# laboshinl/loam_velodyne

Hardware: AMD Instinct MI355X
Metric: sweeps/sec (64-ring, 1M-pt map): feature extraction + odometry + scan-to-map registration (higher is better)
Workload: dtype f32

## Files before the change

### loam_velodyne_amd/csrc/odometry.hip

```cpp
#include "odometry.hpp"
#include "odom_schedule.hpp"
#include "pinned_copy.hpp"
#include <chrono>
#include <cstring>
#include <type_traits>

namespace loamx {

constexpr int OD_THREADS = 256;
constexpr int OD_TR_STRIDE = OD_THREADS + 2;
constexpr int OD_PART_STRIDE = 2 * (2 * 16 * LX_NSUM) + 16;
[[maybe_unused]] constexpr int OD_PART_TS = 2 * (2 * 16 * LX_NSUM);

__device__ inline void sincos_f(float a, float& s, float& c) { sincosf(a, &s, &c); }

__device__ inline void transform_to_start(const float* T, float scan_period, const float4 pi, float& x, float& y, float& z) {
  const float s = (1.f / scan_period) * (pi.w - (float)(int)pi.w);
  x = pi.x - s * T[3];
  y = pi.y - s * T[4];
  z = pi.z - s * T[5];
  float sx, cx, sy, cy, sz, cz;
  sincos_f(-s * T[0], sx, cx);
  sincos_f(-s * T[1], sy, cy);
  sincos_f(-s * T[2], sz, cz);
  rot_z(x, y, cz, sz);
  rot_x(y, z, cx, sx);
  rot_y(x, z, cy, sy);
}

// ... 668 lines not shown
              hm->stats = stt;
              hm->done = done_now;
            }
          }
        }
      }
      LM_TS(9);
    }
    __syncthreads();
    if (sh_done) break;
  }
}

#pragma clang diagnostic pop

__device__ inline float4 to_end_point(float4 p, const ToEndParams& P) {
  const float s = (1.f / P.scan_period) * (p.w - (float)(int)p.w);
  float x = p.x - s * P.T[3], y = p.y - s * P.T[4], z = p.z - s * P.T[5];
  float sx, cx, sy, cy, sz, cz;
  sincos_f(-s * P.T[0], sx, cx);
  sincos_f(-s * P.T[1], sy, cy);
  sincos_f(-s * P.T[2], sz, cz);
  rot_z(x, y, cz, sz); rot_x(y, z, cx, sx); rot_y(x, z, cy, sy);
  rot_y(x, z, P.cT[1], P.sT[1]); rot_x(y, z, P.cT[0], P.sT[0]); rot_z(x, y, P.cT[2], P.sT[2]);
  x += P.T[3] - P.shift[0];
  y += P.T[4] - P.shift[1];
  z += P.T[5] - P.shift[2];
  rot_z(x, y, P.c_start[2], P.s_start[2]); rot_x(y, z, P.c_start[0], P.s_start[0]); rot_y(x, z, P.c_start[1], P.s_start[1]);
  rot_y(x, z, P.c_end[1], -P.s_end[1]); rot_x(y, z, P.c_end[0], -P.s_end[0]); rot_z(x, y, P.c_end[2], -P.s_end[2]);
  return make_float4(x, y, z, (float)(int)p.w);
}
__global__ __launch_bounds__(256) void k_transform_to_end_copy(float4* __restrict__ dst, const float4* __restrict__ src, uint32_t n, ToEndParams P) {
  const uint32_t i = blockIdx.x * blockDim.x + threadIdx.x;
  if (i >= n) return;
  dst[i] = to_end_point(src[i], P);
}
__global__ __launch_bounds__(256) void k_transform_to_end(float4* __restrict__ pts, uint32_t n, ToEndParams P) {
  const uint32_t i = blockIdx.x * blockDim.x + threadIdx.x;
  if (i >= n) return;
  pts[i] = to_end_point(pts[i], P);
}
__global__ void k_te_patch(const OdomProblem* __restrict__ probs, uint32_t na, ToEndParams* __restrict__ te) {
  const uint32_t a = blockIdx.x * blockDim.x + threadIdx.x;
  if (a >= na) return;
  const OdomProblem& pb = probs[a];
  ToEndParams& P = te[pb.stream_id];
// ... 701 lines not shown
```

### loam_velodyne_amd/csrc/odometry.hpp

```cpp
#pragma once
#include "common.h"
#include "host_math.h"
#include "registration.hpp"
#include <atomic>
#include <condition_variable>
#include <functional>
#include <mutex>
#include <thread>

namespace loamx {

struct OdomParams {
  float scan_period = 0.1f;
  int max_iterations = 25;
  float delta_t_abort = 0.1f, delta_r_abort = 0.1f;
};

struct OdomStats {
  int iterations, sel, frame, degenerate;
};

struct ToEndParams;

struct OdomProblem {
  const float4* sharp; uint32_t n_sharp;
  const float4* flat; uint32_t n_flat;
  const float4* last_corner; uint32_t n_last_corner;
  const float4* last_surf; uint32_t n_last_surf;
  const float4* sorted;
  const uint32_t* cell_table;
  const GridDescB* lc_desc;
  const GridDescB* ls_desc;
  int* ind;
  float transform[6];
  OdomStats stats;
  int done;
  float matP[36];
// ... 2 lines not shown
  OdomProblem* host_mirror;
  unsigned ticket;
  unsigned xchg_epoch;
  double* part;
  const uint32_t* rf_corner;
  const uint32_t* rf_surf;
  uint32_t rf_epoch;
  uint32_t* err_word;
};

struct OdomInput {
  const float4* sharp; uint32_t n_sharp;
  const float4* less_sharp; uint32_t n_less_sharp;
  const float4* flat; uint32_t n_flat;
  const float4* less_flat; uint32_t n_less_flat;
};

struct ToEndParams {
  float T[6];
  float sT[3], cT[3];
  float shift[3];
  float s_start[3], c_start[3];
  float s_end[3], c_end[3];
  float scan_period;
  int enabled;
};

constexpr int OD_RF_N = 320;

struct ReprojectProbe {
  int variant;
  float4* pts; uint32_t n;
  const uint32_t* d_off; const uint32_t* h_off; uint32_t K, ns;
  const ToEndParams* d_params; const ToEndParams* h_params;
  const float4* src; const float4* src_s; uint32_t n_corner_all;
  uint32_t* bounds; uint32_t* ring_first; uint32_t rf_epoch;
  const float4* const* table; const uint32_t* sid;
};
void reproject_probe_launch(const ReprojectProbe& a, hipStream_t st);

// ... 112 lines not shown
```

### loam_velodyne_amd/csrc/pipeline.hip

```cpp
#include "pinned_copy.hpp"
#include "features.hpp"
#include "odometry.hpp"
#include "registration.hpp"
#include "hostlink.hpp"
#include "densemap.hpp"
#include "odom_lookahead.hpp"
#include <atomic>
#include <deque>
#include <chrono>
#include <mutex>
#include <memory>

namespace loamx {

struct OdomPub {
  HTwist transform, transform_sum;
  OdomStats stats = {0, 0, 0, 0};
  int rc = LOAMX_SKIPPED;
  const float4* last_corner = nullptr; uint32_t n_last_corner = 0;
  const float4* last_surf = nullptr; uint32_t n_last_surf = 0;
  ToEndParams to_end;
};

struct PipeStreamState {
// ... 75 lines not shown
  uint32_t n_groups = 1;
  std::vector<std::unique_ptr<OdomChain>> chains;
  OdomChain& chain_of(uint32_t s) { uint32_t g = 0; while (g + 1 < n_groups && s >= chains[g]->s1) g++; return *chains[g]; }
  OdometryBatch& OB(uint32_t s) { return *chain_of(s).ob; }
  uint32_t LS(uint32_t s) { return s - chain_of(s).s0; }
  loamx_scanreg_config fcfg;
  uint32_t n_streams_;
  int device;
  std::vector<PipeStreamState> st;
  std::vector<std::unique_ptr<FeatureExtractor>> fx;
  static constexpr uint32_t RING = 8;
  bool streaming = false;
  std::atomic<uint32_t> staged_hi{0};
  hipStream_t cstream = nullptr, dstream = nullptr;
  hipEvent_t ev_stage[RING] = {};
  hipEvent_t ev_reg_done = nullptr, ev_d2h[2] = {nullptr, nullptr};
  bool d2h_pending[2] = {false, false};
  uint64_t downloads_direct = 0, downloads_hip = 0;
  HostLinkDma hostlink;
  HostLinkUp uplink;
  uint32_t up_runs[RING] = {};
  std::atomic<long> last_step{-1};
  std::vector<uint32_t> last_full_off;
  std::vector<uint32_t> last_who;
  struct RawSlot {
    bool raw = false, finalized = true;
    std::vector<uint32_t> count, off;
    DevBuf<char> d_bytes;
    DevBuf<float4> d_raw4, d_binned;
    DevBuf<uint32_t> d_ring_fld;
// ... 58 lines not shown
  float feat_ms[OR] = {};
  int f_hi = -1;
  int ahead_depth = std::max(1, std::min(diag_env("LOAMX_ODOM_AHEAD") ? atoi(diag_env("LOAMX_ODOM_AHEAD")) : 6, OR - 2));
  int depth() const { return !prefetch ? 0 : (streaming ? std::min(ahead_depth, (int)RING - 2) : ahead_depth); }
  float last_ms[4] = {0, 0, 0, 0};
  std::atomic<bool> timing{false};

  std::vector<OdomPub> ores[OR];
  std::unique_ptr<LookAhead> la;
  void run_chain_step(OdomChain& c, uint32_t k) {
    const auto tc0 = std::chrono::steady_clock::now();
    c.tr[0] = tr_us(); run_odometry(c, k); c.tr[3] = tr_us();
    c.last_us.store((float)std::chrono::duration<double, std::micro>(std::chrono::steady_clock::now() - tc0).count(), std::memory_order_relaxed);
  }
  int drain_lookahead() { return prefetch ? la->drain() : la->done_min(); }
  void park_odometry(int restart) {
    if (restart >= 0) pre_t = -1;
    la->park(restart);
  }

  ~Pipeline() {
    la.reset();
    for (auto& c : chains) {
      for (auto& e : c->ev_tail) if (e) (void)hipEventDestroy(e);
      for (auto& tm : c->tm) tm.destroy();
    }
    fx.clear();
    for (auto& a : evF) for (auto& e : a) if (e) (void)hipEventDestroy(e);
    for (auto& tm : tmM) tm.destroy();
    for (auto& e : ev_stage) if (e) (void)hipEventDestroy(e);
    for (auto& r : rawslot) if (r.ev_ingest) (void)hipEventDestroy(r.ev_ingest);
    for (auto& e : ev_d2h) if (e) (void)hipEventDestroy(e);
    if (ev_reg_done) (void)hipEventDestroy(ev_reg_done);
    if (cstream) { (void)hipStreamSynchronize(cstream); (void)hipStreamDestroy(cstream); }
    if (dstream) { (void)hipStreamSynchronize(dstream); (void)hipStreamDestroy(dstream); }
    if (fstream) (void)hipStreamDestroy(fstream);
  }

  void launch_features(uint32_t t) {
    TraceRange trace_range("loamx:features");
    finalize_raw(t);
    FeatureExtractor& F = FX(t);
    const uint32_t ns = n_streams_, nring = F.total_rings();
    if (streaming) {
      LX_HIP(hipStreamWaitEvent(fstream, ev_stage[t % RING], 0));
// ... 6 lines not shown
    F.run_async();
    LX_REQUIRE(F.n_offsets() == 3 * (ns + 1) + nring + 1, "internal: offset table layout");
    store_to_pinned_u32(hb.p, F.d_offsets(), F.n_offsets(), fstream);
    LX_HIP(hipEventRecord(evF[t % OR][1], fstream));
    LA(t) = 1;
  }

  std::unique_ptr<FeatureExtractor> new_extractor_() {
    auto f = std::make_unique<FeatureExtractor>(device, fstream);
    f->params = feat_params_from(fcfg);
    return f;
  }
  void feature_stream_() {
    if (!fstream) fstream = create_stream(env_priority("LOAMX_PRIO_FEAT", -1), diag_env("LOAMX_FEAT_CU_STRIDE") ? atoi(diag_env("LOAMX_FEAT_CU_STRIDE")) : 0, 1);
    LX_HIP(hipStreamSynchronize(fstream));
    fx.clear();
  }
  void restart_input_(uint32_t n_slots, bool ring) {
    streaming = ring;
    staged_hi = 0;
    last_step = -1;
    launched.assign(n_slots, 0);
    la->reset();
    f_hi = -1;
  }

  void upload(uint32_t n_steps, const loamx_cloud* clouds, const uint32_t* const* ring_size, const uint32_t* n_rings) {
    LX_REQUIRE(n_steps >= 1 && clouds && ring_size && n_rings, "invalid argument");
    LX_HIP(hipSetDevice(device));
    feature_stream_();
// ... 1 lines not shown
    for (uint32_t t = 0; t < n_steps; t++) {
      auto f = new_extractor_();
      f->upload(n_streams_, clouds + (size_t)t * n_streams_, ring_size + (size_t)t * n_streams_, n_rings + (size_t)t * n_streams_);
      fx.push_back(std::move(f));
    }
  }

  void begin_staging_(uint32_t t, const char* entry) {
    LX_HIP(hipSetDevice(device));
    if (!streaming) {
      LX_REQUIRE(t == 0, "streaming input starts at step 0");
      feature_stream_();
      for (uint32_t k = 0; k < RING; k++) fx.push_back(new_extractor_());
      if (!cstream) cstream = create_stream(0);
      for (auto& e : ev_stage) if (!e) LX_HIP(hipEventCreateWithFlags(&e, hipEventDisableTiming));
      restart_input_(RING, true);
    }
    LX_REQUIRE(t == staged_hi.load(), "steps must be staged in order");
    LX_REQUIRE(t < RING || last_step.load() + (long)RING >= (long)t, std::string(entry) + "(t) needs step(t - 8) to have run: only eight steps can be in flight");
  }
  void publish_staged_(uint32_t t) {
    LA(t) = 0;
    staged_hi.store(t + 1, std::memory_order_release);
  }

  void stage_step(uint32_t t, const loamx_cloud* clouds, const uint32_t* const* ring_size, const uint32_t* n_rings) {
    LX_REQUIRE(clouds && ring_size && n_rings, "invalid argument");
    begin_staging_(t, "stage_step");
    TraceRange trace_range("loamx:pipeline:stage_step");
    if (t > 0) finalize_raw(t - 1);
    rawslot[t % RING].raw = false;
    rawslot[t % RING].finalized = true;
    static const bool direct = !(diag_env("LOAMX_H2D_DIRECT") && atoi(diag_env("LOAMX_H2D_DIRECT")) == 0);
    const int slot = (int)(t % RING);
// ... 233 lines not shown
    for (auto& tm : c.tm)
      if (tm.resolve()) c.ms.store(tm.ms, std::memory_order_relaxed);
    for (uint32_t s = c.s0; s < c.s1; s++) {
      const uint32_t l = s - c.s0;
      OdomStream& O = odom.stream_state(l);
      OdomPub& N = ores[slot][s];
      N.transform = O.transform;
      N.transform_sum = O.transform_sum;
      N.stats = O.stats;
      N.rc = rc[l];
      N.last_corner = odom.d_last_corner(l); N.n_last_corner = O.n_last_corner;
      N.last_surf = odom.d_last_surf(l); N.n_last_surf = O.n_last_surf;
      N.to_end = odom.to_end_params(l, true);
    }
  }
  int pre_t = -1;
  void prestage_gather(int tn, int last_staged, hipStream_t s_) {
    static const bool off = !(diag_env("LOAMX_PRESTAGE") && atoi(diag_env("LOAMX_PRESTAGE")) != 0);
    if (off || !prefetch || pre_t == tn || tn > last_staged || tn < 1) return;
    const uint32_t ns = n_streams_;
    if (la->done_min() < tn) return;
    FeatureExtractor& F = FX((uint32_t)tn);
    std::vector<const float4*> fsrc;
    std::vector<uint32_t> nfr;
    std::vector<ToEndParams> tep;
    for (uint32_t s = 0; s < ns; s++) {
      const OdomPub& N = ores[tn % OR][s];
      if (N.rc != LOAMX_OK) continue;
      fsrc.push_back(F.d_cloud() + F.point_base(s));
      nfr.push_back(F.point_base(s + 1) - F.point_base(s));
      tep.push_back(N.to_end);
    }
    const uint32_t nw = (uint32_t)fsrc.size();
    if (!nw) return;
    const int par = (int)(run_count & 1);
    hostlink.wait(par);
    if (d2h_pending[par]) { LX_HIP(hipStreamWaitEvent(s_, ev_d2h[par], 0)); d2h_pending[par] = false; }
    float4* dst = reg.stage_full_next(nw, nfr.data());
    if (!dst) return;
    std::vector<uint32_t> foff(nw + 1, 0);
    for (uint32_t k = 0; k < nw; k++) foff[k + 1] = foff[k] + nfr[k];
    chains[0]->ob->to_end_gather(dst, foff.data(), fsrc.data(), tep.data(), nw, s_);
    pre_t = tn;
  }

  bool trace = getenv("LOAMX_PIPE_TRACE") != nullptr;
  std::chrono::steady_clock::time_point tr0, tr_exit = std::chrono::steady_clock::now();
  double tr_us() const { return std::chrono::duration<double, std::micro>(std::chrono::steady_clock::now() - tr0).count(); }

  struct Step {
    uint32_t t = 0;
    int ti = 0, last_staged = -1;
    LookaheadWindow w;
    bool late_pending = false;
    hipStream_t s_ = nullptr;
    std::vector<uint32_t> who;
    std::vector<const float4*> cl, sl, fsrc;
    std::vector<uint32_t> ncl, nsl, nfr;
    std::vector<float> guess;
    std::vector<ToEndParams> to_end;
// ... 57 lines not shown
      const uint32_t k = (uint32_t)S.who.size();
      S.cl[k] = P.cur.last_corner; S.ncl[k] = P.cur.n_last_corner;
      S.sl[k] = P.cur.last_surf; S.nsl[k] = P.cur.n_last_surf;
      S.fsrc[k] = F.d_cloud() + F.point_base(s);
      S.nfr[k] = F.point_base(s + 1) - F.point_base(s);
      S.to_end.push_back(P.cur.to_end);
      S.who.push_back(s);
    }
    S.nw = (uint32_t)S.who.size();
  }
  void stage_full_res_(Step& S) {
    if (!S.nw) { last_full_off.clear(); last_who.clear(); return; }
    const uint32_t nw = S.nw;
    std::vector<uint32_t> foff(nw + 1, 0);
    for (uint32_t k = 0; k < nw; k++) foff[k + 1] = foff[k] + S.nfr[k];
    const bool adopted = pre_t == S.ti && reg.adopt_full_next(nw, S.nfr.data());
    pre_t = -1;
    if (!adopted) {
      if (reg.double_buffer_full) {
        const int par = (int)(run_count & 1);
        const double tw0 = trace ? tr_us() : 0.0;
        hostlink.wait(par);
        if (trace) S.tr[4] = tr_us() - tw0;
        if (d2h_pending[par]) { LX_HIP(hipStreamWaitEvent(S.s_, ev_d2h[par], 0)); d2h_pending[par] = false; }
      }
      float4* full_dst = reg.stage_full(nw, S.nfr.data());
      chains[0]->ob->to_end_gather(full_dst, foff.data(), S.fsrc.data(), S.to_end.data(), nw, S.s_);
    }
    last_full_off = foff;
    last_who = S.who;
    run_count++;
  }
  void enqueue_registration_(Step& S) {
    if (!S.nw) return;
    const uint32_t nw = S.nw;
    const RawSlot& R = rawslot[S.t % RING];
    reg.upload_device(nw, S.cl.data(), S.ncl.data(), S.sl.data(), S.nsl.data(), nullptr, nullptr, S.guess.data());
    bool blend = false;
    static const bool no_blend = diag_env("LOAMX_NO_MAP_IMU_BLEND") != nullptr;
    if (!no_blend && streaming && R.raw && !R.scan_time.empty())
      for (uint32_t k = 0; k < nw; k++) blend = blend || R.map_imu_upto[S.who[k]] > 0;
    reg.defer_full = blend;
    reg.on_first_wait = [&]() { release_late_(S); prestage_gather(S.ti + 1, S.last_staged, S.s_); };
    reg.run_async();
    reg.on_first_wait = nullptr;
    if (blend) {
      std::vector<float> p6(6 * (size_t)nw);
      reg.download(p6.data(), nullptr);
      if (reg.submap_sufficient())
        for (uint32_t k = 0; k < nw; k++)
          (void)map_imu_blend(S.who[k], R.map_imu_upto[S.who[k]], R.scan_time[S.who[k]], fcfg.scan_period, &p6[6 * (size_t)k]);
      reg.finish_with_poses(p6.data());
      reg.defer_full = false;
    }
    if (reg.double_buffer_full) {
      if (!ev_reg_done) LX_HIP(hipEventCreateWithFlags(&ev_reg_done, hipEventDisableTiming));
      LX_HIP(hipEventRecord(ev_reg_done, S.s_));
    }
  }
  void release_behind_registration_(Step& S) {
    release_late_(S);
    if (S.nw) prestage_gather(S.ti + 1, S.last_staged, S.s_);
    if (timing) tmM[S.t & 1].stop(S.s_);
    S.tr[1] = tr_us();
  }
  int collect_(Step& S) {
    int ret = LOAMX_SKIPPED;
    if (S.nw) {
      std::vector<float> poses(6 * (size_t)S.nw);
      std::vector<SweepStats> ss(S.nw);
      reg.download(poses.data(), nullptr);
      reg.download_stats(ss.data());
      for (uint32_t k = 0; k < S.nw; k++) {
        PipeStreamState& P = st[S.who[k]];
        P.map_stats = ss[k];
        P.mapped = true;
        if (reg.submap_sufficient()) {
// ... 292 lines not shown
```

### loam_velodyne_amd/csrc/registration.hip

```cpp
#include "registration.hpp"
#include "pinned_copy.hpp"
#include <atomic>
#include <chrono>
#include "scan.hpp"
#include "voxel.hpp"

namespace loamx {

__global__ __launch_bounds__(256) void k_stack(const float4* __restrict__ in, const float4* const* __restrict__ src, uint32_t n,
                                               const uint32_t* __restrict__ seg_off, uint32_t nseg, const Pose* __restrict__ poses,
                                               float inv_corner, float inv_surf, float4* __restrict__ stack, int* __restrict__ ijk,
                                               int* __restrict__ seg_minmax) {
  const uint32_t i = blockIdx.x * blockDim.x + threadIdx.x;
  const bool active = i < n;
  uint32_t seg = 0;
  int ix = 0, iy = 0, iz = 0;
  if (active) {
    seg = vox_find_seg(seg_off, nseg, i);
    const Pose T = poses[seg >> 1];
    const float4 p = src ? src[seg][i - seg_off[seg]] : in[i];
    float x = p.x, y = p.y, z = p.z;
    to_map(T, x, y, z);
    to_be_mapped(T, x, y, z);
    stack[i] = make_float4(x, y, z, p.w);
// ... 462 lines not shown
  const float4 p = queries[q];
  unsigned long long wk[6];
  uint32_t win[6];
  knn5_group<KNN_LPQ, QB>(*desc, pts, cell_start, p.x, p.y, p.z, gl, tab + grp, wk, win);
  if (gl != 0) return;
#pragma unroll
  for (int j = 0; j < 5; j++) {
    idx5[5 * (size_t)q + j] = wk[j] != KNN_NONE ? (uint32_t)(wk[j] & 0xffffffffull) : 0xffffffffu;
    d2_5[5 * (size_t)q + j] = wk[j] != KNN_NONE ? __uint_as_float((uint32_t)(wk[j] >> 32)) : FLT_MAX;
  }
}

__global__ __launch_bounds__(256) void k_transform_full(float4* __restrict__ full, uint32_t n, const uint32_t* __restrict__ full_off,
                                                        uint32_t ns, const Pose* __restrict__ poses, const SweepStats* __restrict__ stats,
                                                        uint32_t* __restrict__ full_done, int mode, uint32_t tag,
                                                        const uint32_t* __restrict__ skip_word, uint32_t skip_value) {
  uint32_t i = blockIdx.x * blockDim.x + threadIdx.x;
  if (i >= n) return;
  if (skip_word && *skip_word == skip_value) return;
  const uint32_t s = vox_find_seg(full_off, ns, i);
  if (mode == 1) {
    if (!stats[s].done) return;
    if (i == full_off[s]) full_done[s] = tag;
  } else if (mode == 2) {
    if (full_done[s] != 0u) return;
  }
  const Pose T = poses[s];
  float4 p = full[i];
  to_map(T, p.x, p.y, p.z);
  full[i] = p;
}

__global__ __launch_bounds__(256) void k_gather_segments(float4* __restrict__ dst, const uint32_t* __restrict__ off, uint32_t nseg,
                                                         const float4* const* __restrict__ src, uint32_t n) {
  const uint32_t i = blockIdx.x * blockDim.x + threadIdx.x;
  if (i >= n) return;
  const uint32_t k = vox_find_seg(off, nseg, i);
  dst[i] = src[k][i - off[k]];
}

struct ParamBlock1 { uint32_t w[18]; };
__global__ __launch_bounds__(256) void k_gather_one(float4* __restrict__ dst, const float4* __restrict__ src, uint32_t n, ParamBlock1 blk,
                                                    uint32_t* __restrict__ blk_dst) {
// ... 109 lines not shown
  LX_HIP(hipStreamWaitEvent(st_, ev_build_, 0));
  LX_HIP(hipEventRecord(ev_swap_, st_));
  corner_index.swap(corner_next_);
  surf_index.swap(surf_next_);
  corner_index.bind(st_);
  surf_index.bind(st_);
  next_staged_ = false;
  swapped_once_ = true;
}

template <class Count> static void prefix_offsets(std::vector<uint32_t>& off, uint32_t n, Count&& count) {
  off.assign(n + 1, 0);
  for (uint32_t s = 0; s < n; s++) off[s + 1] = off[s] + count(s);
}

template <class Count> void Registrar::plan_inputs_(uint32_t n_sweeps, bool staged, Count&& count) {
  LX_REQUIRE(n_sweeps >= 1 && n_sweeps <= max_sweeps_, "n_sweeps out of range for this handle");
  LX_HIP(hipSetDevice(device_));
  n_sweeps_ = n_sweeps;
  h_seg_off_.assign(2 * n_sweeps + 1, 0);
  if (!staged) h_full_off_.assign(n_sweeps + 1, 0);
  max_q_per_sweep_ = 0;
  for (uint32_t s = 0; s < n_sweeps; s++) {
    const uint32_t nc = count(s, 0), nf = count(s, 1);
    h_seg_off_[2 * s + 1] = h_seg_off_[2 * s] + nc;
    h_seg_off_[2 * s + 2] = h_seg_off_[2 * s + 1] + nf;
    max_q_per_sweep_ = std::max(max_q_per_sweep_, nc + nf);
    if (!staged) h_full_off_[s + 1] = h_full_off_[s] + count(s, 2);
  }
  n_in_ = h_seg_off_[2 * n_sweeps];
  if (!staged) n_full_ = h_full_off_[n_sweeps];
  in_.reserve(n_in_ + 1);
  stack_.reserve(n_in_ + 1);
  ds_pts_.reserve(n_in_ + 1);
  vox_.reserve(n_in_ + 1, 2 * n_sweeps);
  LX_REQUIRE(n_in_ < SCAN_MAX_N, "too many feature points in one batch");
  if (n_full_) full_.reserve(n_full_);
  nblk_ = max_q_per_sweep_ / GN_TILE + 2;
  partials_.reserve((size_t)n_sweeps * nblk_ * LX_NSUM);
}

size_t Registrar::write_param_block_(const float* guess6, const float4* const* corner_src, const float4* const* surf_src, const float4* const* full_src) {
  const uint32_t ns = n_sweeps_;
  const size_t nseg = 2 * (size_t)ns;
  const size_t o_off = sizeof(float) * 6 * ns, o_full = o_off + sizeof(uint32_t) * (nseg + 1);
  const size_t end_full = o_full + sizeof(uint32_t) * (ns + 1), o_src = (end_full + 15) & ~(size_t)15;
  const size_t bytes = corner_src ? o_src + sizeof(float4*) * (nseg + ns) : end_full;
  h_blob_.reserve(bytes + 16);
  blob_.reserve(bytes + 16);
  memcpy(h_blob_.p, guess6, sizeof(float) * 6 * ns);
  memcpy(h_blob_.p + o_off, h_seg_off_.data(), sizeof(uint32_t) * (nseg + 1));
  memcpy(h_blob_.p + o_full, h_full_off_.data(), sizeof(uint32_t) * (ns + 1));
  if (corner_src) {
    const float4** hsrc = (const float4**)(h_blob_.p + o_src);
    for (uint32_t s = 0; s < ns; s++) { hsrc[2 * s] = corner_src[s]; hsrc[2 * s + 1] = surf_src[s]; }
    for (uint32_t s = 0; s < ns; s++) hsrc[nseg + s] = full_src ? full_src[s] : nullptr;
  }
  d_guess_ = (const float*)blob_.p;
  d_seg_off_ = (const uint32_t*)(blob_.p + o_off);
  d_full_off_ = (const uint32_t*)(blob_.p + o_full);
  d_src_ = corner_src ? (const float4* const*)(blob_.p + o_src) : nullptr;
  return bytes;
}

void Registrar::upload(uint32_t n_sweeps, const loamx_cloud* corner_last, const loamx_cloud* surf_last, const loamx_cloud* full_res,
                       const float* guess6, bool wait) {
  LX_REQUIRE(corner_last && surf_last && guess6, "NULL input");
  plan_inputs_(n_sweeps, false, [&](uint32_t s, int k) {
    const loamx_cloud* c = k == 0 ? &corner_last[s] : k == 1 ? &surf_last[s] : full_res ? &full_res[s] : nullptr;
    if (!c) return 0u;
    check_cloud(c, false);
    return c->count;
  });
  h_in_.reserve(n_in_ + 1);
  for (uint32_t s = 0; s < n_sweeps; s++) {
    pack_cloud(&corner_last[s], h_in_.p + h_seg_off_[2 * s]);
    pack_cloud(&surf_last[s], h_in_.p + h_seg_off_[2 * s + 1]);
  }
  if (!packed_all_finite(h_in_.p, n_in_)) throw Error(LOAMX_E_INVALID, "a feature cloud holds non-finite coordinates");
  fetch_from_pinned(in_.p, h_in_.p, n_in_, st_);
  if (n_full_) {
    h_full_.reserve(n_full_);
    for (uint32_t s = 0; s < n_sweeps; s++) pack_cloud(&full_res[s], h_full_.p + h_full_off_[s]);
    fetch_from_pinned(full_.p, h_full_.p, n_full_, st_);
  }
  const size_t bytes = write_param_block_(guess6, nullptr, nullptr, nullptr);
  LX_HIP(hipMemcpyAsync(blob_.p, h_blob_.p, bytes, hipMemcpyHostToDevice, st_));
  if (wait) LX_HIP(hipStreamSynchronize(st_));
}

float4* Registrar::stage_full(uint32_t n_sweeps, const uint32_t* n_full) {
  LX_REQUIRE(n_sweeps >= 1 && n_sweeps <= max_sweeps_, "n_sweeps out of range for this handle");
  full_next_staged_ = false;
  prefix_offsets(h_full_off_, n_sweeps, [&](uint32_t s) { return n_full[s]; });
  n_full_ = h_full_off_[n_sweeps];
  if (double_buffer_full) {
    std::swap(full_.p, full_alt_.p);
    std::swap(full_.cap, full_alt_.cap);
  }
  full_.reserve((size_t)n_full_ + 1);
  full_staged_ = true;
  return full_.p;
}

float4* Registrar::stage_full_next(uint32_t n_sweeps, const uint32_t* n_full) {
  LX_REQUIRE(double_buffer_full, "internal: pre-staging needs the second full-resolution buffer");
  LX_REQUIRE(n_sweeps >= 1 && n_sweeps <= max_sweeps_, "n_sweeps out of range for this handle");
  prefix_offsets(next_full_off_, n_sweeps, [&](uint32_t s) { return n_full[s]; });
  if ((size_t)next_full_off_[n_sweeps] + 1 > full_alt_.cap) return nullptr;
  full_next_staged_ = true;
  return full_alt_.p;
}
bool Registrar::adopt_full_next(uint32_t n_sweeps, const uint32_t* n_full) {
  if (!full_next_staged_ || next_full_off_.size() != n_sweeps + 1) { full_next_staged_ = false; return false; }
  for (uint32_t s = 0; s < n_sweeps; s++)
    if (next_full_off_[s + 1] - next_full_off_[s] != n_full[s]) { full_next_staged_ = false; return false; }
  full_next_staged_ = false;
  h_full_off_ = next_full_off_;
  n_full_ = h_full_off_[n_sweeps];
  std::swap(full_.p, full_alt_.p);
  std::swap(full_.cap, full_alt_.cap);
  full_staged_ = true;
  return true;
}

void Registrar::upload_device(uint32_t n_sweeps, const float4* const* corner_last, const uint32_t* n_corner,
                              const float4* const* surf_last, const uint32_t* n_surf, const float4* const* full_res,
                              const uint32_t* n_full, const float* guess6) {
  const bool staged = full_staged_ && !full_res;
  full_staged_ = false;
  plan_inputs_(n_sweeps, staged, [&](uint32_t s, int k) { return k == 0 ? n_corner[s] : k == 1 ? n_surf[s] : full_res ? n_full[s] : 0u; });
  const size_t bytes = write_param_block_(guess6, corner_last, surf_last, full_res);
  if (n_sweeps == 1 && n_full_ && !staged && bytes == sizeof(ParamBlock1)) {
    ParamBlock1 pb1;
    memcpy(pb1.w, h_blob_.p, sizeof(pb1));
    hipLaunchKernelGGL(k_gather_one, dim3((n_full_ + 255) / 256), dim3(256), 0, st_, full_.p, full_res[0], n_full_, pb1, (uint32_t*)blob_.p);
  } else {
    LX_HIP(hipMemcpyAsync(blob_.p, h_blob_.p, bytes, hipMemcpyHostToDevice, st_));
    if (n_full_ && !staged)
      hipLaunchKernelGGL(k_gather_segments, dim3((n_full_ + 255) / 256), dim3(256), 0, st_, full_.p, d_full_off_, n_sweeps, d_src_ + 2 * (size_t)n_sweeps,
                         n_full_);
  }
}

static double host_us() {
  return std::chrono::duration<double, std::micro>(std::chrono::steady_clock::now().time_since_epoch()).count();
}
struct Registrar::RunTrace {
  bool on;
  double t0, front = 0, first_gn = 0, callback = 0;
  int looks = 0;
};
#ifdef LOAMX_PROF_GN
static DevBuf<unsigned long long> g_gn_dbg;
#endif

void Registrar::enqueue_full(int mode) {
  if (!n_full_) return;
  if (mode == 1 && ++full_tag_ == 0u) full_tag_ = 1u;
  const uint32_t* skip = run_.vb_unchecked ? vb_.d_fail_word() : nullptr;
  hipLaunchKernelGGL(k_transform_full, dim3((n_full_ + 255) / 256), dim3(256), 0, st_, full_.p, n_full_, d_full_off_, n_sweeps_, poses_.p,
                     stats_.p, full_done_.p, mode, full_tag_, skip, vb_.epoch());
}

void Registrar::enqueue_front(bool legacy) {
  const uint32_t ns = n_sweeps_, nseg = 2 * ns, n = n_in_;
  if (legacy || n == 0)
    hipLaunchKernelGGL(k_pose_init, dim3((ns + 63) / 64), dim3(64), 0, st_, d_guess_, ns, poses_.p, stats_.p, vox_.seg_minmax(), arrive_.p,
                       full_done_.p);
  if (n == 0) {
    LX_HIP(hipMemsetAsync(ds_off_.p, 0, sizeof(uint32_t) * (nseg + 1), st_));
    return;
  }
  if (legacy) {
    const uint32_t nb = (n + 255) / 256;
    hipLaunchKernelGGL(k_stack, dim3(nb), dim3(256), 0, st_, in_.p, d_src_, n, d_seg_off_, nseg, poses_.p, 1.0f / params.corner_leaf,
                       1.0f / params.surf_leaf, stack_.p, vox_.ijk(), vox_.seg_minmax());
// ... 416 lines not shown
```

### loam_velodyne_amd/csrc/registration.hpp

```cpp
#pragma once
#include <functional>
#include "common.h"
#include "dev_math.hpp"
#include "reg_schedule.hpp"
#include "submap_index.hpp"
#include "voxel.hpp"
#include "voxbucket.hpp"

namespace loamx {

constexpr int LX_RES_THREADS = 256;
constexpr int LX_NSUM = 28;

struct SweepStats {
  int iterations, sel, corner_q, surf_q, degenerate, done, pad0, pad1;
};

__host__ __device__ inline int mirror_check_word(const SweepStats& st, const Pose& T) {
  const unsigned* w = reinterpret_cast<const unsigned*>(&T);
  unsigned x = 0x5bd1e995u ^ (unsigned)st.iterations ^ ((unsigned)st.sel << 8) ^ ((unsigned)st.degenerate << 30);
  for (int i = 0; i < (int)(sizeof(Pose) / 4); i++) x = (x << 5 | x >> 27) ^ w[i];
  return (int)x;
}

// ... 14 lines not shown
  bool submap_staged() const { return next_staged_; }
  void swap_submap();
  bool double_buffer_full = false;
  bool defer_full = false;
  void finish_with_poses(const float* poses6);
  std::function<void()> on_first_wait;
  bool early_exit = false;
  hipStream_t stream() const { return st_; }

  void set_submap_host(const loamx_cloud* corner, const loamx_cloud* surf);
  void set_submap_device(const float4* d_corner, uint32_t nc, const float4* d_surf, uint32_t ns, bool sync = true);

  void upload(uint32_t n_sweeps, const loamx_cloud* corner_last, const loamx_cloud* surf_last, const loamx_cloud* full_res,
              const float* guess6, bool wait = true);
  void upload_device(uint32_t n_sweeps, const float4* const* corner_last, const uint32_t* n_corner, const float4* const* surf_last,
                     const uint32_t* n_surf, const float4* const* full_res, const uint32_t* n_full, const float* guess6);
  float4* stage_full(uint32_t n_sweeps, const uint32_t* n_full);
  float4* stage_full_next(uint32_t n_sweeps, const uint32_t* n_full);
  bool adopt_full_next(uint32_t n_sweeps, const uint32_t* n_full);
  void run_async(bool force_general = false);
  void sync();
  void download(float* poses6, int* stats4);
  void download_stats(SweepStats* out);
  int download_full_res(uint32_t sweep, loamx_cloud* out);
  void download_full_res_async(uint32_t sweep, const loamx_cloud* into = nullptr);
  void set_submap_device_split(const float4* d_corner, uint32_t nc, hipStream_t corner_stream, const float4* d_surf, uint32_t ns, bool bounds_done = false);
  void download_ds(uint32_t sweep, std::vector<float4>& corner_ds, std::vector<float4>& surf_ds);
  void download_ds_counts(uint32_t sweep, uint32_t counts[2]);
  const float4* d_ds_points() const { return ds_pts_.p; }
  const uint32_t* d_ds_offsets() const { return ds_off_.p; }
  const Pose* d_poses() const { return poses_.p; }
  const float4* d_full_res() const { return full_.p; }
  uint32_t full_offset(uint32_t s) const { return h_full_off_[s]; }

// ... 7 lines not shown

 private:
  int device_;
  uint32_t max_sweeps_, n_sweeps_ = 0;
  hipStream_t st_ = nullptr;
  bool timing_ = false, timed_run_ = false, launch_timing_ = true;

  DevBuf<float4> own_corner_, own_surf_;

  PinBuf<float4> h_in_, h_full_;
  std::vector<uint32_t> h_seg_off_, h_full_off_;
  PinBuf<float> h_guess_;
  DevBuf<float4> in_, stack_, ds_pts_, full_, full_alt_;
  DevBuf<uint32_t> ds_off_;
  DevBuf<float> guess_;
  bool full_staged_ = false, full_next_staged_ = false;
  std::vector<uint32_t> next_full_off_;
  hipEvent_t ev_look_ = nullptr;
  PinBuf<float4> h_full_dl_;
  struct Run {
    bool vb_unchecked = false;
    bool mirrors_written = false;
    bool results_final = false;
    int full_dl_sweep = -1;
    void* full_dl_direct = nullptr;
  } run_;
  VoxelPipeline vox_;
  VoxBucket vb_;
  bool vb_disabled_ = false;
  bool jacobi_eig_ = false;
  void enqueue_front(bool legacy);
  void enqueue_full(int mode);
  void redo_if_bucket_path_failed();
  uint32_t n_in_ = 0, n_full_ = 0, max_q_per_sweep_ = 0;
  struct RunTrace;
  template <class Count> void plan_inputs_(uint32_t n_sweeps, bool staged, Count&& count);
  size_t write_param_block_(const float* guess6, const float4* const* corner_src, const float4* const* surf_src, const float4* const* full_src);
  void begin_attempt_(bool legacy);
  RegOutcome run_iterations(RunTrace& tr);
  bool bucket_stage_gave_up_();
  void dump_gn_profile_();
  bool wait_for_mirrors();
  void fetch_results();
  int pred_iters_ = 4;

  DevBuf<Pose> poses_;
  DevBuf<SweepStats> stats_;
  DevBuf<float> matP_;
  DevBuf<double> partials_;
  const float* d_guess_ = nullptr;
  const uint32_t* d_seg_off_ = nullptr;
  const uint32_t* d_full_off_ = nullptr;
  const float4* const* d_src_ = nullptr;
  DevBuf<char> blob_;
  PinBuf<char> h_blob_;
  SubMapIndex corner_next_, surf_next_;
  DevBuf<float4> next_corner_, next_surf_;
  PinBuf<float4> h_next_corner_, h_next_surf_;
  hipStream_t st_build_ = nullptr;
  hipEvent_t ev_build_ = nullptr, ev_swap_ = nullptr;
  bool next_staged_ = false, swapped_once_ = false;
  DevBuf<uint32_t> arrive_;
  DevBuf<uint32_t> full_done_;
  uint32_t full_tag_ = 0;
  uint32_t nblk_ = 0;

  std::vector<hipEvent_t> ev_;
  int n_res_launch_ = 0;
// ... 6 lines not shown
```

Baseline: 16730.

## Fuse full-res to-end reprojection into map transform kernel, drop prestage gather

Before, the full-resolution cloud was gathered and reprojected to the sweep end in a separate to_end_gather pass into a staged buffer. That pass could optionally be prestaged for the next step. Now k_transform_full reads each point straight from the feature extractor's cloud, applies to_end_point and then the map pose in one kernel. This removes a separate launch and a full write/read round trip of the cloud. In exchange, the source clouds must stay alive until registration finishes, so new ev_src_read events and extra stream syncs hold back ring-slot reuse, which may add host stalls.

After: 17060, median of 6. 1.02x the previous value.

```diff
diff --git a/loam_velodyne_amd/csrc/odometry.hip b/loam_velodyne_amd/csrc/odometry.hip
--- a/loam_velodyne_amd/csrc/odometry.hip
+++ b/loam_velodyne_amd/csrc/odometry.hip
@@ -11,8 +11,6 @@
 constexpr int OD_TR_STRIDE = OD_THREADS + 2;
 constexpr int OD_PART_STRIDE = 2 * (2 * 16 * LX_NSUM) + 16;
 [[maybe_unused]] constexpr int OD_PART_TS = 2 * (2 * 16 * LX_NSUM);
-
-__device__ inline void sincos_f(float a, float& s, float& c) { sincosf(a, &s, &c); }
 
 __device__ inline void transform_to_start(const float* T, float scan_period, const float4 pi, float& x, float& y, float& z) {
   const float s = (1.f / scan_period) * (pi.w - (float)(int)pi.w);
@@ -711,22 +709,6 @@
 
 #pragma clang diagnostic pop
 
-__device__ inline float4 to_end_point(float4 p, const ToEndParams& P) {
-  const float s = (1.f / P.scan_period) * (p.w - (float)(int)p.w);
-  float x = p.x - s * P.T[3], y = p.y - s * P.T[4], z = p.z - s * P.T[5];
-  float sx, cx, sy, cy, sz, cz;
-  sincos_f(-s * P.T[0], sx, cx);
-  sincos_f(-s * P.T[1], sy, cy);
-  sincos_f(-s * P.T[2], sz, cz);
-  rot_z(x, y, cz, sz); rot_x(y, z, cx, sx); rot_y(x, z, cy, sy);
-  rot_y(x, z, P.cT[1], P.sT[1]); rot_x(y, z, P.cT[0], P.sT[0]); rot_z(x, y, P.cT[2], P.sT[2]);
-  x += P.T[3] - P.shift[0];
-  y += P.T[4] - P.shift[1];
-  z += P.T[5] - P.shift[2];
-  rot_z(x, y, P.c_start[2], P.s_start[2]); rot_x(y, z, P.c_start[0], P.s_start[0]); rot_y(x, z, P.c_start[1], P.s_start[1]);
-  rot_y(x, z, P.c_end[1], -P.s_end[1]); rot_x(y, z, P.c_end[0], -P.s_end[0]); rot_z(x, y, P.c_end[2], -P.s_end[2]);
-  return make_float4(x, y, z, (float)(int)p.w);
-}
 __global__ __launch_bounds__(256) void k_transform_to_end_copy(float4* __restrict__ dst, const float4* __restrict__ src, uint32_t n, ToEndParams P) {
   const uint32_t i = blockIdx.x * blockDim.x + threadIdx.x;
   if (i >= n) return;
diff --git a/loam_velodyne_amd/csrc/odometry.hpp b/loam_velodyne_amd/csrc/odometry.hpp
--- a/loam_velodyne_amd/csrc/odometry.hpp
+++ b/loam_velodyne_amd/csrc/odometry.hpp
@@ -2,6 +2,7 @@
 #include "common.h"
 #include "host_math.h"
 #include "registration.hpp"
+#include "to_end.hpp"
 #include <atomic>
 #include <condition_variable>
 #include <functional>
@@ -19,8 +20,6 @@
 struct OdomStats {
   int iterations, sel, frame, degenerate;
 };
-
-struct ToEndParams;
 
 struct OdomProblem {
   const float4* sharp; uint32_t n_sharp;
@@ -53,16 +52,6 @@
   const float4* less_sharp; uint32_t n_less_sharp;
   const float4* flat; uint32_t n_flat;
   const float4* less_flat; uint32_t n_less_flat;
-};
-
-struct ToEndParams {
-  float T[6];
-  float sT[3], cT[3];
-  float shift[3];
-  float s_start[3], c_start[3];
-  float s_end[3], c_end[3];
-  float scan_period;
-  int enabled;
 };
 
 constexpr int OD_RF_N = 320;
diff --git a/loam_velodyne_amd/csrc/pipeline.hip b/loam_velodyne_amd/csrc/pipeline.hip
--- a/loam_velodyne_amd/csrc/pipeline.hip
+++ b/loam_velodyne_amd/csrc/pipeline.hip
@@ -113,6 +113,7 @@
   std::atomic<uint32_t> staged_hi{0};
   hipStream_t cstream = nullptr, dstream = nullptr;
   hipEvent_t ev_stage[RING] = {};
+  hipEvent_t ev_src_read[RING] = {};
   hipEvent_t ev_reg_done = nullptr, ev_d2h[2] = {nullptr, nullptr};
   bool d2h_pending[2] = {false, false};
   uint64_t downloads_direct = 0, downloads_hip = 0;
@@ -201,10 +202,7 @@
     c.last_us.store((float)std::chrono::duration<double, std::micro>(std::chrono::steady_clock::now() - tc0).count(), std::memory_order_relaxed);
   }
   int drain_lookahead() { return prefetch ? la->drain() : la->done_min(); }
-  void park_odometry(int restart) {
-    if (restart >= 0) pre_t = -1;
-    la->park(restart);
-  }
+  void park_odometry(int restart) { la->park(restart); }
 
   ~Pipeline() {
     la.reset();
@@ -212,10 +210,12 @@
       for (auto& e : c->ev_tail) if (e) (void)hipEventDestroy(e);
       for (auto& tm : c->tm) tm.destroy();
     }
+    (void)hipStreamSynchronize(reg.stream());
     fx.clear();
     for (auto& a : evF) for (auto& e : a) if (e) (void)hipEventDestroy(e);
     for (auto& tm : tmM) tm.destroy();
     for (auto& e : ev_stage) if (e) (void)hipEventDestroy(e);
+    for (auto& e : ev_src_read) if (e) (void)hipEventDestroy(e);
     for (auto& r : rawslot) if (r.ev_ingest) (void)hipEventDestroy(r.ev_ingest);
     for (auto& e : ev_d2h) if (e) (void)hipEventDestroy(e);
     if (ev_reg_done) (void)hipEventDestroy(ev_reg_done);
@@ -252,6 +252,7 @@
   void feature_stream_() {
     if (!fstream) fstream = create_stream(env_priority("LOAMX_PRIO_FEAT", -1), diag_env("LOAMX_FEAT_CU_STRIDE") ? atoi(diag_env("LOAMX_FEAT_CU_STRIDE")) : 0, 1);
     LX_HIP(hipStreamSynchronize(fstream));
+    LX_HIP(hipStreamSynchronize(reg.stream()));
     fx.clear();
   }
   void restart_input_(uint32_t n_slots, bool ring) {
@@ -283,10 +284,12 @@
       for (uint32_t k = 0; k < RING; k++) fx.push_back(new_extractor_());
       if (!cstream) cstream = create_stream(0);
       for (auto& e : ev_stage) if (!e) LX_HIP(hipEventCreateWithFlags(&e, hipEventDisableTiming));
+      for (auto& e : ev_src_read) if (!e) LX_HIP(hipEventCreateWithFlags(&e, hipEventDisableTiming));
       restart_input_(RING, true);
     }
     LX_REQUIRE(t == staged_hi.load(), "steps must be staged in order");
     LX_REQUIRE(t < RING || last_step.load() + (long)RING >= (long)t, std::string(entry) + "(t) needs step(t - 8) to have run: only eight steps can be in flight");
+    if (t >= RING) LX_HIP(hipEventSynchronize(ev_src_read[t % RING]));
   }
   void publish_staged_(uint32_t t) {
     LA(t) = 0;
@@ -550,36 +553,6 @@
       N.to_end = odom.to_end_params(l, true);
     }
   }
-  int pre_t = -1;
-  void prestage_gather(int tn, int last_staged, hipStream_t s_) {
-    static const bool off = !(diag_env("LOAMX_PRESTAGE") && atoi(diag_env("LOAMX_PRESTAGE")) != 0);
-    if (off || !prefetch || pre_t == tn || tn > last_staged || tn < 1) return;
-    const uint32_t ns = n_streams_;
-    if (la->done_min() < tn) return;
-    FeatureExtractor& F = FX((uint32_t)tn);
-    std::vector<const float4*> fsrc;
-    std::vector<uint32_t> nfr;
-    std::vector<ToEndParams> tep;
-    for (uint32_t s = 0; s < ns; s++) {
-      const OdomPub& N = ores[tn % OR][s];
-      if (N.rc != LOAMX_OK) continue;
-      fsrc.push_back(F.d_cloud() + F.point_base(s));
-      nfr.push_back(F.point_base(s + 1) - F.point_base(s));
-      tep.push_back(N.to_end);
-    }
-    const uint32_t nw = (uint32_t)fsrc.size();
-    if (!nw) return;
-    const int par = (int)(run_count & 1);
-    hostlink.wait(par);
-    if (d2h_pending[par]) { LX_HIP(hipStreamWaitEvent(s_, ev_d2h[par], 0)); d2h_pending[par] = false; }
-    float4* dst = reg.stage_full_next(nw, nfr.data());
-    if (!dst) return;
-    std::vector<uint32_t> foff(nw + 1, 0);
-    for (uint32_t k = 0; k < nw; k++) foff[k + 1] = foff[k] + nfr[k];
-    chains[0]->ob->to_end_gather(dst, foff.data(), fsrc.data(), tep.data(), nw, s_);
-    pre_t = tn;
-  }
-
   bool trace = getenv("LOAMX_PIPE_TRACE") != nullptr;
   std::chrono::steady_clock::time_point tr0, tr_exit = std::chrono::steady_clock::now();
   double tr_us() const { return std::chrono::duration<double, std::micro>(std::chrono::steady_clock::now() - tr0).count(); }
@@ -667,18 +640,12 @@
     const uint32_t nw = S.nw;
     std::vector<uint32_t> foff(nw + 1, 0);
     for (uint32_t k = 0; k < nw; k++) foff[k + 1] = foff[k] + S.nfr[k];
-    const bool adopted = pre_t == S.ti && reg.adopt_full_next(nw, S.nfr.data());
-    pre_t = -1;
-    if (!adopted) {
-      if (reg.double_buffer_full) {
-        const int par = (int)(run_count & 1);
-        const double tw0 = trace ? tr_us() : 0.0;
-        hostlink.wait(par);
-        if (trace) S.tr[4] = tr_us() - tw0;
-        if (d2h_pending[par]) { LX_HIP(hipStreamWaitEvent(S.s_, ev_d2h[par], 0)); d2h_pending[par] = false; }
-      }
-      float4* full_dst = reg.stage_full(nw, S.nfr.data());
-      chains[0]->ob->to_end_gather(full_dst, foff.data(), S.fsrc.data(), S.to_end.data(), nw, S.s_);
+    if (reg.double_buffer_full) {
+      const int par = (int)(run_count & 1);
+      const double tw0 = trace ? tr_us() : 0.0;
+      hostlink.wait(par);
+      if (trace) S.tr[4] = tr_us() - tw0;
+      if (d2h_pending[par]) { LX_HIP(hipStreamWaitEvent(S.s_, ev_d2h[par], 0)); d2h_pending[par] = false; }
     }
     last_full_off = foff;
     last_who = S.who;
@@ -688,13 +655,13 @@
     if (!S.nw) return;
     const uint32_t nw = S.nw;
     const RawSlot& R = rawslot[S.t % RING];
-    reg.upload_device(nw, S.cl.data(), S.ncl.data(), S.sl.data(), S.nsl.data(), nullptr, nullptr, S.guess.data());
+    reg.upload_device(nw, S.cl.data(), S.ncl.data(), S.sl.data(), S.nsl.data(), S.fsrc.data(), S.nfr.data(), S.guess.data(), S.to_end.data());
     bool blend = false;
     static const bool no_blend = diag_env("LOAMX_NO_MAP_IMU_BLEND") != nullptr;
     if (!no_blend && streaming && R.raw && !R.scan_time.empty())
       for (uint32_t k = 0; k < nw; k++) blend = blend || R.map_imu_upto[S.who[k]] > 0;
     reg.defer_full = blend;
-    reg.on_first_wait = [&]() { release_late_(S); prestage_gather(S.ti + 1, S.last_staged, S.s_); };
+    reg.on_first_wait = [&]() { release_late_(S); };
     reg.run_async();
     reg.on_first_wait = nullptr;
     if (blend) {
@@ -710,10 +677,10 @@
       if (!ev_reg_done) LX_HIP(hipEventCreateWithFlags(&ev_reg_done, hipEventDisableTiming));
       LX_HIP(hipEventRecord(ev_reg_done, S.s_));
     }
+    if (streaming) LX_HIP(hipEventRecord(ev_src_read[S.t % RING], S.s_));
   }
   void release_behind_registration_(Step& S) {
     release_late_(S);
-    if (S.nw) prestage_gather(S.ti + 1, S.last_staged, S.s_);
     if (timing) tmM[S.t & 1].stop(S.s_);
     S.tr[1] = tr_us();
   }
diff --git a/loam_velodyne_amd/csrc/registration.hip b/loam_velodyne_amd/csrc/registration.hip
--- a/loam_velodyne_amd/csrc/registration.hip
+++ b/loam_velodyne_amd/csrc/registration.hip
@@ -500,7 +500,8 @@
 __global__ __launch_bounds__(256) void k_transform_full(float4* __restrict__ full, uint32_t n, const uint32_t* __restrict__ full_off,
                                                         uint32_t ns, const Pose* __restrict__ poses, const SweepStats* __restrict__ stats,
                                                         uint32_t* __restrict__ full_done, int mode, uint32_t tag,
-                                                        const uint32_t* __restrict__ skip_word, uint32_t skip_value) {
+                                                        const uint32_t* __restrict__ skip_word, uint32_t skip_value,
+                                                        const float4* const* __restrict__ src, const ToEndParams* __restrict__ te) {
   uint32_t i = blockIdx.x * blockDim.x + threadIdx.x;
   if (i >= n) return;
   if (skip_word && *skip_word == skip_value) return;
@@ -512,7 +513,7 @@
     if (full_done[s] != 0u) return;
   }
   const Pose T = poses[s];
-  float4 p = full[i];
+  float4 p = src ? to_end_point(src[s][i - full_off[s]], te[s]) : full[i];
   to_map(T, p.x, p.y, p.z);
   full[i] = p;
 }
@@ -652,38 +653,45 @@
   for (uint32_t s = 0; s < n; s++) off[s + 1] = off[s] + count(s);
 }
 
-template <class Count> void Registrar::plan_inputs_(uint32_t n_sweeps, bool staged, Count&& count) {
+template <class Count> void Registrar::plan_inputs_(uint32_t n_sweeps, bool fused, Count&& count) {
   LX_REQUIRE(n_sweeps >= 1 && n_sweeps <= max_sweeps_, "n_sweeps out of range for this handle");
   LX_HIP(hipSetDevice(device_));
   n_sweeps_ = n_sweeps;
   h_seg_off_.assign(2 * n_sweeps + 1, 0);
-  if (!staged) h_full_off_.assign(n_sweeps + 1, 0);
+  h_full_off_.assign(n_sweeps + 1, 0);
   max_q_per_sweep_ = 0;
   for (uint32_t s = 0; s < n_sweeps; s++) {
     const uint32_t nc = count(s, 0), nf = count(s, 1);
     h_seg_off_[2 * s + 1] = h_seg_off_[2 * s] + nc;
     h_seg_off_[2 * s + 2] = h_seg_off_[2 * s + 1] + nf;
     max_q_per_sweep_ = std::max(max_q_per_sweep_, nc + nf);
-    if (!staged) h_full_off_[s + 1] = h_full_off_[s] + count(s, 2);
+    h_full_off_[s + 1] = h_full_off_[s] + count(s, 2);
   }
   n_in_ = h_seg_off_[2 * n_sweeps];
-  if (!staged) n_full_ = h_full_off_[n_sweeps];
+  n_full_ = h_full_off_[n_sweeps];
   in_.reserve(n_in_ + 1);
   stack_.reserve(n_in_ + 1);
   ds_pts_.reserve(n_in_ + 1);
   vox_.reserve(n_in_ + 1, 2 * n_sweeps);
   LX_REQUIRE(n_in_ < SCAN_MAX_N, "too many feature points in one batch");
-  if (n_full_) full_.reserve(n_full_);
+  full_fused_ = fused;
+  if (fused && double_buffer_full) {
+    std::swap(full_.p, full_alt_.p);
+    std::swap(full_.cap, full_alt_.cap);
+  }
+  if (n_full_) full_.reserve((size_t)n_full_ + 1);
   nblk_ = max_q_per_sweep_ / GN_TILE + 2;
   partials_.reserve((size_t)n_sweeps * nblk_ * LX_NSUM);
 }
 
-size_t Registrar::write_param_block_(const float* guess6, const float4* const* corner_src, const float4* const* surf_src, const float4* const* full_src) {
+size_t Registrar::write_param_block_(const float* guess6, const float4* const* corner_src, const float4* const* surf_src, const float4* const* full_src,
+                                     const ToEndParams* full_to_end) {
   const uint32_t ns = n_sweeps_;
   const size_t nseg = 2 * (size_t)ns;
   const size_t o_off = sizeof(float) * 6 * ns, o_full = o_off + sizeof(uint32_t) * (nseg + 1);
   const size_t end_full = o_full + sizeof(uint32_t) * (ns + 1), o_src = (end_full + 15) & ~(size_t)15;
-  const size_t bytes = corner_src ? o_src + sizeof(float4*) * (nseg + ns) : end_full;
+  const size_t o_te = o_src + sizeof(float4*) * (nseg + ns);
+  const size_t bytes = !corner_src ? end_full : full_to_end ? o_te + sizeof(ToEndParams) * ns : o_te;
   h_blob_.reserve(bytes + 16);
   blob_.reserve(bytes + 16);
   memcpy(h_blob_.p, guess6, sizeof(float) * 6 * ns);
@@ -693,11 +701,13 @@
     const float4** hsrc = (const float4**)(h_blob_.p + o_src);
     for (uint32_t s = 0; s < ns; s++) { hsrc[2 * s] = corner_src[s]; hsrc[2 * s + 1] = surf_src[s]; }
     for (uint32_t s = 0; s < ns; s++) hsrc[nseg + s] = full_src ? full_src[s] : nullptr;
+    if (full_to_end) memcpy(h_blob_.p + o_te, full_to_end, sizeof(ToEndParams) * ns);
   }
   d_guess_ = (const float*)blob_.p;
   d_seg_off_ = (const uint32_t*)(blob_.p + o_off);
   d_full_off_ = (const uint32_t*)(blob_.p + o_full);
   d_src_ = corner_src ? (const float4* const*)(blob_.p + o_src) : nullptr;
+  d_full_te_ = corner_src && full_to_end ? (const ToEndParams*)(blob_.p + o_te) : nullptr;
   return bytes;
 }
 
@@ -722,60 +732,25 @@
     for (uint32_t s = 0; s < n_sweeps; s++) pack_cloud(&full_res[s], h_full_.p + h_full_off_[s]);
     fetch_from_pinned(full_.p, h_full_.p, n_full_, st_);
   }
-  const size_t bytes = write_param_block_(guess6, nullptr, nullptr, nullptr);
+  const size_t bytes = write_param_block_(guess6, nullptr, nullptr, nullptr, nullptr);
   LX_HIP(hipMemcpyAsync(blob_.p, h_blob_.p, bytes, hipMemcpyHostToDevice, st_));
   if (wait) LX_HIP(hipStreamSynchronize(st_));
 }
 
-float4* Registrar::stage_full(uint32_t n_sweeps, const uint32_t* n_full) {
-  LX_REQUIRE(n_sweeps >= 1 && n_sweeps <= max_sweeps_, "n_sweeps out of range for this handle");
-  full_next_staged_ = false;
-  prefix_offsets(h_full_off_, n_sweeps, [&](uint32_t s) { return n_full[s]; });
-  n_full_ = h_full_off_[n_sweeps];
-  if (double_buffer_full) {
-    std::swap(full_.p, full_alt_.p);
-    std::swap(full_.cap, full_alt_.cap);
-  }
-  full_.reserve((size_t)n_full_ + 1);
-  full_staged_ = true;
-  return full_.p;
-}
-
-float4* Registrar::stage_full_next(uint32_t n_sweeps, const uint32_t* n_full) {
-  LX_REQUIRE(double_buffer_full, "internal: pre-staging needs the second full-resolution buffer");
-  LX_REQUIRE(n_sweeps >= 1 && n_sweeps <= max_sweeps_, "n_sweeps out of range for this handle");
-  prefix_offsets(next_full_off_, n_sweeps, [&](uint32_t s) { return n_full[s]; });
-  if ((size_t)next_full_off_[n_sweeps] + 1 > full_alt_.cap) return nullptr;
-  full_next_staged_ = true;
-  return full_alt_.p;
-}
-bool Registrar::adopt_full_next(uint32_t n_sweeps, const uint32_t* n_full) {
-  if (!full_next_staged_ || next_full_off_.size() != n_sweeps + 1) { full_next_staged_ = false; return false; }
-  for (uint32_t s = 0; s < n_sweeps; s++)
-    if (next_full_off_[s + 1] - next_full_off_[s] != n_full[s]) { full_next_staged_ = false; return false; }
-  full_next_staged_ = false;
-  h_full_off_ = next_full_off_;
-  n_full_ = h_full_off_[n_sweeps];
-  std::swap(full_.p, full_alt_.p);
-  std::swap(full_.cap, full_alt_.cap);
-  full_staged_ = true;
-  return true;
-}
-
 void Registrar::upload_device(uint32_t n_sweeps, const float4* const* corner_last, const uint32_t* n_corner,
                               const float4* const* surf_last, const uint32_t* n_surf, const float4* const* full_res,
-                              const uint32_t* n_full, const float* guess6) {
-  const bool staged = full_staged_ && !full_res;
-  full_staged_ = false;
-  plan_inputs_(n_sweeps, staged, [&](uint32_t s, int k) { return k == 0 ? n_corner[s] : k == 1 ? n_surf[s] : full_res ? n_full[s] : 0u; });
-  const size_t bytes = write_param_block_(guess6, corner_last, surf_last, full_res);
-  if (n_sweeps == 1 && n_full_ && !staged && bytes == sizeof(ParamBlock1)) {
+                              const uint32_t* n_full, const float* guess6, const ToEndParams* full_to_end) {
+  const bool fused = full_res && full_to_end;
+  LX_REQUIRE(full_res || !full_to_end, "re-projection parameters without full-resolution clouds");
+  plan_inputs_(n_sweeps, fused, [&](uint32_t s, int k) { return k == 0 ? n_corner[s] : k == 1 ? n_surf[s] : full_res ? n_full[s] : 0u; });
+  const size_t bytes = write_param_block_(guess6, corner_last, surf_last, full_res, full_to_end);
+  if (n_sweeps == 1 && n_full_ && !fused && bytes == sizeof(ParamBlock1)) {
     ParamBlock1 pb1;
     memcpy(pb1.w, h_blob_.p, sizeof(pb1));
     hipLaunchKernelGGL(k_gather_one, dim3((n_full_ + 255) / 256), dim3(256), 0, st_, full_.p, full_res[0], n_full_, pb1, (uint32_t*)blob_.p);
   } else {
     LX_HIP(hipMemcpyAsync(blob_.p, h_blob_.p, bytes, hipMemcpyHostToDevice, st_));
-    if (n_full_ && !staged)
+    if (n_full_ && !fused)
       hipLaunchKernelGGL(k_gather_segments, dim3((n_full_ + 255) / 256), dim3(256), 0, st_, full_.p, d_full_off_, n_sweeps, d_src_ + 2 * (size_t)n_sweeps,
                          n_full_);
   }
@@ -798,7 +773,8 @@
   if (mode == 1 && ++full_tag_ == 0u) full_tag_ = 1u;
   const uint32_t* skip = run_.vb_unchecked ? vb_.d_fail_word() : nullptr;
   hipLaunchKernelGGL(k_transform_full, dim3((n_full_ + 255) / 256), dim3(256), 0, st_, full_.p, n_full_, d_full_off_, n_sweeps_, poses_.p,
-                     stats_.p, full_done_.p, mode, full_tag_, skip, vb_.epoch());
+                     stats_.p, full_done_.p, mode, full_tag_, skip, vb_.epoch(), full_fused_ ? d_src_ + 2 * (size_t)n_sweeps_ : nullptr,
+                     full_fused_ ? d_full_te_ : nullptr);
 }
 
 void Registrar::enqueue_front(bool legacy) {
diff --git a/loam_velodyne_amd/csrc/registration.hpp b/loam_velodyne_amd/csrc/registration.hpp
--- a/loam_velodyne_amd/csrc/registration.hpp
+++ b/loam_velodyne_amd/csrc/registration.hpp
@@ -3,6 +3,7 @@
 #include "common.h"
 #include "dev_math.hpp"
 #include "reg_schedule.hpp"
+#include "to_end.hpp"
 #include "submap_index.hpp"
 #include "voxel.hpp"
 #include "voxbucket.hpp"
@@ -52,10 +53,8 @@
   void upload(uint32_t n_sweeps, const loamx_cloud* corner_last, const loamx_cloud* surf_last, const loamx_cloud* full_res,
               const float* guess6, bool wait = true);
   void upload_device(uint32_t n_sweeps, const float4* const* corner_last, const uint32_t* n_corner, const float4* const* surf_last,
-                     const uint32_t* n_surf, const float4* const* full_res, const uint32_t* n_full, const float* guess6);
-  float4* stage_full(uint32_t n_sweeps, const uint32_t* n_full);
-  float4* stage_full_next(uint32_t n_sweeps, const uint32_t* n_full);
-  bool adopt_full_next(uint32_t n_sweeps, const uint32_t* n_full);
+                     const uint32_t* n_surf, const float4* const* full_res, const uint32_t* n_full, const float* guess6,
+                     const ToEndParams* full_to_end = nullptr);
   void run_async(bool force_general = false);
   void sync();
   void download(float* poses6, int* stats4);
@@ -93,8 +92,7 @@
   DevBuf<float4> in_, stack_, ds_pts_, full_, full_alt_;
   DevBuf<uint32_t> ds_off_;
   DevBuf<float> guess_;
-  bool full_staged_ = false, full_next_staged_ = false;
-  std::vector<uint32_t> next_full_off_;
+  bool full_fused_ = false;
   hipEvent_t ev_look_ = nullptr;
   PinBuf<float4> h_full_dl_;
   struct Run {
@@ -113,8 +111,9 @@
   void redo_if_bucket_path_failed();
   uint32_t n_in_ = 0, n_full_ = 0, max_q_per_sweep_ = 0;
   struct RunTrace;
-  template <class Count> void plan_inputs_(uint32_t n_sweeps, bool staged, Count&& count);
-  size_t write_param_block_(const float* guess6, const float4* const* corner_src, const float4* const* surf_src, const float4* const* full_src);
+  template <class Count> void plan_inputs_(uint32_t n_sweeps, bool fused, Count&& count);
+  size_t write_param_block_(const float* guess6, const float4* const* corner_src, const float4* const* surf_src, const float4* const* full_src,
+                            const ToEndParams* full_to_end);
   void begin_attempt_(bool legacy);
   RegOutcome run_iterations(RunTrace& tr);
   bool bucket_stage_gave_up_();
@@ -131,6 +130,7 @@
   const uint32_t* d_seg_off_ = nullptr;
   const uint32_t* d_full_off_ = nullptr;
   const float4* const* d_src_ = nullptr;
+  const ToEndParams* d_full_te_ = nullptr;
   DevBuf<char> blob_;
   PinBuf<char> h_blob_;
   SubMapIndex corner_next_, surf_next_;
diff --git a/loam_velodyne_amd/csrc/to_end.hpp b/loam_velodyne_amd/csrc/to_end.hpp
--- /dev/null
+++ b/loam_velodyne_amd/csrc/to_end.hpp
@@ -0,0 +1,35 @@
+#pragma once
+#include "dev_math.hpp"
+
+namespace loamx {
+
+struct ToEndParams {
+  float T[6];
+  float sT[3], cT[3];
+  float shift[3];
+  float s_start[3], c_start[3];
+  float s_end[3], c_end[3];
+  float scan_period;
+  int enabled;
+};
+
+__device__ inline void sincos_f(float a, float& s, float& c) { sincosf(a, &s, &c); }
+
+__device__ inline float4 to_end_point(float4 p, const ToEndParams& P) {
+  const float s = (1.f / P.scan_period) * (p.w - (float)(int)p.w);
+  float x = p.x - s * P.T[3], y = p.y - s * P.T[4], z = p.z - s * P.T[5];
+  float sx, cx, sy, cy, sz, cz;
+  sincos_f(-s * P.T[0], sx, cx);
+  sincos_f(-s * P.T[1], sy, cy);
+  sincos_f(-s * P.T[2], sz, cz);
+  rot_z(x, y, cz, sz); rot_x(y, z, cx, sx); rot_y(x, z, cy, sy);
+  rot_y(x, z, P.cT[1], P.sT[1]); rot_x(y, z, P.cT[0], P.sT[0]); rot_z(x, y, P.cT[2], P.sT[2]);
+  x += P.T[3] - P.shift[0];
+  y += P.T[4] - P.shift[1];
+  z += P.T[5] - P.shift[2];
+  rot_z(x, y, P.c_start[2], P.s_start[2]); rot_x(y, z, P.c_start[0], P.s_start[0]); rot_y(x, z, P.c_start[1], P.s_start[1]);
+  rot_y(x, z, P.c_end[1], -P.s_end[1]); rot_x(y, z, P.c_end[0], -P.s_end[0]); rot_z(x, y, P.c_end[2], -P.s_end[2]);
+  return make_float4(x, y, z, (float)(int)p.w);
+}
+
+}
```
